# laclouis5/StructureDetector

Measured on AMD Instinct MI355X. Metric: images/sec (train fwd+bwd) and decode us/img at 512x512, higher is better.
Workload: dtype f32

## Files before the change

include/sdnet_hip.h:

```cpp
#ifndef SDNET_HIP_H
#define SDNET_HIP_H

#include <stddef.h>
#include <stdint.h>

#ifdef __cplusplus
extern "C" {
#endif

#define SD_ERR_INVALID   (-1)
#define SD_ERR_WORKSPACE (-2)
#define SD_ERR_ALIGN     (-3)

#define SD_MAX_TOPK 1024

typedef void* sd_stream_t;

int         sd_version(void);
const char* sd_last_error(void);
int         sd_build_flags(void);


int sd_clamped_sigmoid(const float* x, float* y, int64_t n, sd_stream_t stream);

// ... 198 lines not shown
int sd_loss_fwd_per_image(const sd_loss_desc* d, float* out, void* workspace, size_t workspace_bytes, sd_stream_t stream);

int sd_loss_bwd(const sd_loss_desc* d, const float* out8, const float* grad_out, float* dhead, sd_stream_t stream);



typedef struct sd_conv_desc {
    int B, Hi, Wi, Cin, Ho, Wo, Cout, R, S, stride, pad;
} sd_conv_desc;

size_t sd_conv2d_fwd_workspace_bytes(const sd_conv_desc* d);
int sd_conv2d_fwd(const float* x_nhwc, const float* w_krsc, float* y_nhwc, const sd_conv_desc* d,
                  const float* scale, const float* shift, const float* residual, int res_up2, int relu,
                  void* workspace, size_t workspace_bytes, sd_stream_t stream);
size_t sd_conv2d_stem_fwd_workspace_bytes(const sd_conv_desc* d);
int sd_conv2d_stem_fwd(const float* x_nchw, const float* w_krsc, void* y_nhwc, const sd_conv_desc* d,
                       const float* scale, const float* shift, int relu, int out_bf16, void* workspace,
                       size_t workspace_bytes, sd_stream_t stream);

int    sd_conv2d_fwd_sb_supported(const sd_conv_desc* d, int bf16);
size_t sd_conv2d_fwd_sb_workspace_bytes(const sd_conv_desc* d, int bf16);
size_t sd_conv2d_fwd_sb_state_bytes(const sd_conv_desc* d, int bf16);
int sd_conv2d_fwd_sb(const void* x_nhwc, const void* w_krsc, void* y_nhwc, const sd_conv_desc* d, const float* scale, const float* shift,
                     const void* residual, int res_up2, int relu, int bf16, void* workspace, size_t workspace_bytes, void* state,
                     size_t state_bytes, sd_stream_t stream);

size_t sd_conv2d_stem_fwd_bn_stats_workspace_bytes(const sd_conv_desc* d);
int sd_conv2d_stem_fwd_bn_stats(const float* x_nchw, const float* w, float* y, const sd_conv_desc* d, float eps, float momentum,
                                float* running_mean, float* running_var, float* mean, float* invstd, void* workspace,
                                size_t workspace_bytes, sd_stream_t stream);

size_t sd_conv2d_fwd_bn_stats_workspace_bytes(const sd_conv_desc* d);
int sd_conv2d_fwd_bn_stats(const float* x, const float* w, float* y, const sd_conv_desc* d, float eps, float momentum,
                           float* running_mean, float* running_var, float* mean, float* invstd, void* workspace,
                           size_t workspace_bytes, sd_stream_t stream);
int sd_bn_finalize_scratch_rows(int rows);
int sd_bn_finalize_stats(const float* partial, int rows, int64_t M, int C, float eps, float momentum, float* running_mean,
                         float* running_var, float* mean, float* invstd, float* scratch, sd_stream_t stream);

size_t sd_conv2d_dgrad_bn_reduce_workspace_bytes(const sd_conv_desc* d);
int sd_conv2d_dgrad_bn_reduce(const float* dy, const float* w_t, float* dx, const sd_conv_desc* d, const float* residual,
                              const float* bn_x, const float* bn_y, int relu, const float* mean, const float* invstd,
                              const float* gamma, const float* beta, float* dgamma, float* dbeta, int accumulate,
                              float* means_out, void* workspace, size_t workspace_bytes, sd_stream_t stream);
int sd_bn_bwd_finalize(const float* partial, int rows, int64_t M, int C, float* dgamma, float* dbeta, int accumulate,
                       float* means_out, float* scratch, sd_stream_t stream);
int sd_bn_bwd_apply(const float* dy, const float* x, const float* y, int relu, int64_t M, int C, const float* mean,
                    const float* invstd, const float* gamma, const float* beta, const float* means, float* dx, float* g_out,
                    sd_stream_t stream);

int sd_set_option(const char* name, int value);

const char* sd_conv2d_kernel_name(const sd_conv_desc* d, int pass);

int sd_cast_f32_to_bf16(const float* x, void* y_bf16, int64_t n, sd_stream_t stream);
size_t sd_conv2d_fwd_bf16_workspace_bytes(const sd_conv_desc* d);
int sd_conv2d_fwd_bf16(const void* x_nhwc_bf16, const void* w_krsc_bf16, void* y_nhwc_bf16, const sd_conv_desc* d,
                       const float* scale, const float* shift, const void* residual_bf16, int res_up2, int relu,
                       void* workspace, size_t workspace_bytes, sd_stream_t stream);
int sd_maxpool3x3s2_fwd_bf16(const void* x_bf16, void* y_bf16, int B, int Hi, int Wi, int C, sd_stream_t stream);
int sd_stem_bn_relu_maxpool_fwd_bf16(const float* x_nchw, const float* w, const float* scale, const float* shift, void* y_bf16,
                                     const sd_conv_desc* d, sd_stream_t stream);

int sd_cast_bf16_to_f32(const void* x_bf16, float* y, int64_t n, sd_stream_t stream);
size_t sd_conv2d_fwd_bf16_bn_stats_workspace_bytes(const sd_conv_desc* d);
int sd_conv2d_fwd_bf16_bn_stats(const void* x_nhwc_bf16, const void* w_krsc_bf16, void* y_nhwc_bf16, const sd_conv_desc* d, float eps,
                                float momentum, float* running_mean, float* running_var, float* mean, float* invstd,
                                void* workspace, size_t workspace_bytes, sd_stream_t stream);
int sd_conv2d_stem_fwd_bn_stats_bf16mm(const float* x_nchw, const float* w, float* y, const sd_conv_desc* d, float eps, float momentum,
                                       float* running_mean, float* running_var, float* mean, float* invstd,
                                       void* workspace, size_t workspace_bytes, sd_stream_t stream);
int sd_conv2d_stem_fwd_bn_stats_bf16(const float* x_nchw, const float* w, void* y_bf16, const sd_conv_desc* d, float eps, float momentum,
                                     float* running_mean, float* running_var, float* mean, float* invstd, void* workspace,
                                     size_t workspace_bytes, sd_stream_t stream);
int sd_bn_relu_maxpool_fwd_bf16(const void* x_bf16, int B, int Hi, int Wi, int C, const float* mean, const float* invstd, const float* gamma,
                                const float* beta, void* y_pool_bf16, uint8_t* idx, sd_stream_t stream);
int sd_maxpool_bn_relu_bwd_bf16(const void* dpool_bf16, const uint8_t* idx, const void* x_bf16, int B, int Hi, int Wi, int C, const float* mean,
                                const float* invstd, const float* gamma, const float* beta, float* dx, float* dgamma, float* dbeta, int accumulate,
                                void* workspace, size_t workspace_bytes, sd_stream_t stream);
int sd_maxpool_bn_relu_bwd_bf16_dx16(const void* dpool_bf16, const uint8_t* idx, const void* x_bf16, int B, int Hi, int Wi, int C, const float* mean,
                                     const float* invstd, const float* gamma, const float* beta, void* dx_bf16, float* dgamma, float* dbeta,
                                     int accumulate, void* workspace, size_t workspace_bytes, sd_stream_t stream);
int sd_conv2d_transpose_weights_bf16(const float* w, void* w_t_bf16, int Cout, int taps, int Cin, sd_stream_t stream);

int sd_conv2d_fwd_bf16_head_supported(const sd_conv_desc* d, int head_co);
size_t sd_head_split_bf16_bytes(void);
int sd_head_split_bf16(const float* head_w, const float* head_bias, int head_co, void* prepared, sd_stream_t stream);
int sd_conv2d_fwd_bf16_head(const void* x_bf16, const void* w_bf16, const sd_conv_desc* d, const float* scale, const float* shift, int relu,
                            const void* head_prepared, int head_co, float* head_y, sd_stream_t stream);
int sd_conv2d_dgrad_bf16(const void* dy_bf16, const void* w_t_bf16, void* dx_bf16, const sd_conv_desc* d, const void* residual_bf16,
                         int res_mode, sd_stream_t stream);
size_t sd_conv2d_wgrad_bf16_workspace_bytes(const sd_conv_desc* d);
int sd_conv2d_wgrad_bf16(const void* dy_bf16, const void* x_nhwc_bf16, float* dw_krsc, const sd_conv_desc* d, int accumulate,
                         void* workspace, size_t workspace_bytes, sd_stream_t stream);
int sd_bn_apply_bf16(const void* x, void* y, int64_t M, int C, const float* mean, const float* invstd, const float* gamma,
                     const float* beta, const void* residual, int relu, uint8_t* relu_mask_out, sd_stream_t stream);
int sd_bn_bwd_bf16(const void* dy, const void* x, const void* y, int relu, int64_t M, int C, const float* mean, const float* invstd,
                   const float* gamma, const float* beta, void* dx, void* g_out, float* dgamma, float* dbeta, int accumulate,
                   void* workspace, size_t workspace_bytes, sd_stream_t stream);
int sd_bn_train_stats_bf16(const void* x, int64_t M, int C, float eps, float momentum, float* running_mean, float* running_var,
                           float* mean, float* invstd, void* workspace, size_t workspace_bytes, sd_stream_t stream);
int sd_col_sum_bf16(const void* x, int64_t M, int C, float* out, int accumulate, void* workspace, size_t workspace_bytes, sd_stream_t stream);
int sd_upsample2x_bwd_bf16(const void* dy, const void* add, void* dx, int B, int H, int W, int C, sd_stream_t stream);
int sd_head_fwd_bf16(const void* x_nhwc_bf16, const float* w, const float* bias, float* y_nchw, int B, int HW, int C,
                     int Co, sd_stream_t stream);
int sd_conv2d_dgrad(const float* dy_nhwc, const float* w_t, float* dx_nhwc, const sd_conv_desc* d,
// ... 129 lines not shown
```

structuredetector_amd/_lib.py:

```python
from __future__ import annotations

import ctypes as C
import os
from pathlib import Path

import torch

_HERE = Path(__file__).resolve().parent
LIB_PATH = Path(os.environ.get("SDNET_HIP_LIB", _HERE / "csrc" / "libsdnet_hip.so"))

_lib = None

c_f32p = C.c_void_p
c_i64 = C.c_int64
c_int = C.c_int
c_float = C.c_float
c_size = C.c_size_t
c_vp = C.c_void_p


class SdError(RuntimeError):
    pass


# ... 104 lines not shown
    "sd_conv2d_fwd_sb": (c_int, [c_vp, c_vp, c_vp, C.POINTER(ConvDesc), c_vp, c_vp, c_vp, c_int, c_int, c_int, c_vp, c_size, c_vp, c_size, c_vp]),
    "sd_conv2d_stem_fwd_workspace_bytes": (c_size, [C.POINTER(ConvDesc)]),
    "sd_conv2d_stem_fwd": (c_int, [c_vp, c_vp, c_vp, C.POINTER(ConvDesc), c_vp, c_vp, c_int, c_int, c_vp, c_size, c_vp]),
    "sd_cast_f32_to_bf16": (c_int, [c_vp, c_vp, c_i64, c_vp]),
    "sd_conv2d_fwd_bf16_workspace_bytes": (c_size, [C.POINTER(ConvDesc)]),
    "sd_conv2d_fwd_bf16": (c_int, [c_vp, c_vp, c_vp, C.POINTER(ConvDesc), c_vp, c_vp, c_vp, c_int, c_int, c_vp, c_size, c_vp]),
    "sd_conv2d_fwd_bf16_head_supported": (c_int, [C.POINTER(ConvDesc), c_int]),
    "sd_head_split_bf16_bytes": (c_size, []),
    "sd_head_split_bf16": (c_int, [c_vp, c_vp, c_int, c_vp, c_vp]),
    "sd_conv2d_fwd_bf16_head": (c_int, [c_vp, c_vp, C.POINTER(ConvDesc), c_vp, c_vp, c_int, c_vp, c_int, c_vp, c_vp]),
    "sd_cast_bf16_to_f32": (c_int, [c_vp, c_vp, c_i64, c_vp]),
    "sd_conv2d_fwd_bf16_bn_stats_workspace_bytes": (c_size, [c_vp]),
    "sd_conv2d_fwd_bf16_bn_stats": (c_int, [c_vp, c_vp, c_vp, c_vp, c_float, c_float, c_vp, c_vp, c_vp, c_vp, c_vp, c_size, c_vp]),
    "sd_conv2d_wgrad_bf16_workspace_bytes": (c_size, [c_vp]),
    "sd_conv2d_wgrad_bf16": (c_int, [c_vp, c_vp, c_vp, c_vp, c_int, c_vp, c_size, c_vp]),
    "sd_conv2d_transpose_weights_bf16": (c_int, [c_vp, c_vp, c_int, c_int, c_int, c_vp]),
    "sd_conv2d_dgrad_bf16": (c_int, [c_vp, c_vp, c_vp, c_vp, c_vp, c_int, c_vp]),
    "sd_bn_apply_bf16": (c_int, [c_vp, c_vp, c_i64, c_int, c_vp, c_vp, c_vp, c_vp, c_vp, c_int, c_vp, c_vp]),
    "sd_bn_bwd_bf16": (c_int, [c_vp, c_vp, c_vp, c_int, c_i64, c_int, c_vp, c_vp, c_vp, c_vp, c_vp, c_vp, c_vp, c_vp, c_int, c_vp, c_size, c_vp]),
    "sd_bn_train_stats_bf16": (c_int, [c_vp, c_i64, c_int, c_float, c_float, c_vp, c_vp, c_vp, c_vp, c_vp, c_size, c_vp]),
    "sd_col_sum_bf16": (c_int, [c_vp, c_i64, c_int, c_vp, c_int, c_vp, c_size, c_vp]),
    "sd_upsample2x_bwd_bf16": (c_int, [c_vp, c_vp, c_vp, c_int, c_int, c_int, c_int, c_vp]),
    "sd_maxpool3x3s2_fwd_bf16": (c_int, [c_vp, c_vp, c_int, c_int, c_int, c_int, c_vp]),
    "sd_stem_bn_relu_maxpool_fwd_bf16": (c_int, [c_vp, c_vp, c_vp, c_vp, c_vp, c_vp, c_vp]),
    "sd_head_fwd_bf16": (c_int, [c_vp, c_vp, c_vp, c_vp, c_int, c_int, c_int, c_int, c_vp]),
    "sd_conv2d_dgrad": (c_int, [c_vp, c_vp, c_vp, C.POINTER(ConvDesc), c_vp, c_vp]),
    "sd_conv2d_transpose_weights": (c_int, [c_vp, c_vp, c_int, c_int, c_int, c_vp]),
    "sd_conv2d_transpose_weights_batched": (c_int, [c_vp, c_vp, c_vp, c_int, c_int, c_int, c_vp]),
    "sd_conv2d_wgrad_workspace_bytes": (c_size, [C.POINTER(ConvDesc)]),
    "sd_conv2d_wgrad": (c_int, [c_vp, c_vp, c_vp, C.POINTER(ConvDesc), c_int, c_vp, c_size, c_vp]),
    "sd_conv2d_stem_wgrad_workspace_bytes": (c_size, [C.POINTER(ConvDesc)]),
    "sd_conv2d_stem_wgrad": (c_int, [c_vp, c_vp, c_vp, C.POINTER(ConvDesc), c_int, c_vp, c_size, c_vp]),
    "sd_conv2d_stem_wgrad_bf16mm": (c_int, [c_vp, c_vp, c_vp, C.POINTER(ConvDesc), c_int, c_vp, c_size, c_vp]),
    "sd_conv2d_stem_wgrad_bf16": (c_int, [c_vp, c_vp, c_vp, C.POINTER(ConvDesc), c_int, c_vp, c_size, c_vp]),
    "sd_col_reduce_workspace_bytes": (c_size, [c_i64, c_int]),
    "sd_bn_train_stats": (c_int, [c_vp, c_i64, c_int, c_float, c_float, c_vp, c_vp, c_vp, c_vp, c_vp, c_size, c_vp]),
    "sd_bn_apply": (c_int, [c_vp, c_vp, c_i64, c_int, c_vp, c_vp, c_vp, c_vp, c_vp, c_int, c_vp, c_vp]),
    "sd_bn_fold": (c_int, [c_vp, c_vp, c_vp, c_vp, c_float, c_int, c_vp, c_vp, c_vp]),
    "sd_bn_bwd": (c_int, [c_vp, c_vp, c_vp, c_int, c_i64, c_int, c_vp, c_vp, c_vp, c_vp, c_vp, c_vp, c_vp, c_vp, c_int, c_vp, c_size, c_vp]),
    "sd_col_sum": (c_int, [c_vp, c_i64, c_int, c_vp, c_int, c_vp, c_size, c_vp]),
    "sd_maxpool3x3s2_fwd": (c_int, [c_vp, c_vp, c_vp, c_int, c_int, c_int, c_int, c_vp]),
    "sd_maxpool3x3s2_bwd": (c_int, [c_vp, c_vp, c_vp, c_int, c_int, c_int, c_int, c_vp]),
    "sd_upsample2x_bwd": (c_int, [c_vp, c_vp, c_vp, c_int, c_int, c_int, c_int, c_vp]),
    "sd_head_fwd": (c_int, [c_vp, c_vp, c_vp, c_vp, c_int, c_int, c_int, c_int, c_vp]),
    "sd_head_bwd_workspace_bytes": (c_size, [c_int] * 4),
    "sd_head_bwd": (c_int, [c_vp] * 6 + [c_int] * 5 + [c_vp, c_size, c_vp]),
    "sd_head_bwd_bf16": (c_int, [c_vp] * 6 + [c_int] * 5 + [c_vp, c_size, c_vp]),
    "sd_adam_step": (c_int, [c_vp, c_vp, c_vp, c_vp, c_i64, c_int, c_float, c_float, c_float, c_float, c_float, c_vp]),
    "sd_grad_sumsq_workspace_bytes": (c_size, [c_i64]),
    "sd_grad_sumsq": (c_int, [c_vp, c_i64, c_vp, c_size, c_vp]),
    "sd_optim_step": (c_int, [c_vp, c_vp, c_vp, c_vp, c_i64, c_int, c_float, c_float, c_float, c_float, c_float, c_float, c_vp, c_float, c_vp, c_int,
                              c_vp, c_float, c_vp, c_vp]),
    "sd_conv2d_kernel_name": (C.c_char_p, [c_vp, c_int]),
    "sd_set_option": (c_int, [C.c_char_p, c_int]),
    "sd_decode_set_option": (c_int, [C.c_char_p, c_int]),
    "sd_decode_kernel_names": (C.c_char_p, [c_int] * 9),
    "sd_conv2d_stem_fwd_bn_stats_workspace_bytes": (c_size, [c_vp]),
    "sd_conv2d_stem_fwd_bn_stats": (c_int, [c_vp, c_vp, c_vp, c_vp, c_float, c_float, c_vp, c_vp, c_vp, c_vp, c_vp, c_size, c_vp]),
    "sd_conv2d_stem_fwd_bn_stats_bf16mm": (c_int, [c_vp, c_vp, c_vp, c_vp, c_float, c_float, c_vp, c_vp, c_vp, c_vp, c_vp, c_size, c_vp]),
    "sd_conv2d_stem_fwd_bn_stats_bf16": (c_int, [c_vp, c_vp, c_vp, c_vp, c_float, c_float, c_vp, c_vp, c_vp, c_vp, c_vp, c_size, c_vp]),
    "sd_conv2d_dgrad_half_res": (c_int, [c_vp] * 6),
    "sd_bn_relu_maxpool_fwd": (c_int, [c_vp, c_int, c_int, c_int, c_int] + [c_vp] * 7),
    "sd_bn_relu_maxpool_fwd_bf16": (c_int, [c_vp, c_int, c_int, c_int, c_int] + [c_vp] * 7),
    "sd_maxpool_bn_relu_bwd": (c_int, [c_vp, c_vp, c_vp, c_int, c_int, c_int, c_int] + [c_vp] * 7 + [c_int, c_vp, c_size, c_vp]),
    "sd_maxpool_bn_relu_bwd_bf16": (c_int, [c_vp, c_vp, c_vp, c_int, c_int, c_int, c_int] + [c_vp] * 7 + [c_int, c_vp, c_size, c_vp]),
    "sd_maxpool_bn_relu_bwd_bf16_dx16": (c_int, [c_vp, c_vp, c_vp, c_int, c_int, c_int, c_int] + [c_vp] * 7 + [c_int, c_vp, c_size, c_vp]),
    "sd_conv2d_fwd_bn_stats_workspace_bytes": (c_size, [c_vp]),
    "sd_conv2d_fwd_bn_stats": (c_int, [c_vp, c_vp, c_vp, c_vp, c_float, c_float, c_vp, c_vp, c_vp, c_vp, c_vp, c_size, c_vp]),
    "sd_conv2d_dgrad_bn_reduce_workspace_bytes": (c_size, [c_vp]),
    "sd_conv2d_dgrad_bn_reduce": (c_int, [c_vp] * 5 + [c_vp, c_vp, c_int] + [c_vp] * 6 + [c_int, c_vp, c_vp, c_size, c_vp]),
    "sd_bn_bwd_finalize": (c_int, [c_vp, c_int, c_i64, c_int, c_vp, c_vp, c_int, c_vp, c_vp, c_vp]),
    "sd_bn_bwd_apply": (c_int, [c_vp, c_vp, c_vp, c_int, c_i64, c_int] + [c_vp] * 8),
    "sd_bn_finalize_scratch_rows": (c_int, [c_int]),
    "sd_bn_finalize_stats": (c_int, [c_vp, c_int, c_i64, c_int, c_float, c_float, c_vp, c_vp, c_vp, c_vp, c_vp, c_vp]),
    "sd_bn_stats_from_sums": (c_int, [c_vp, c_int, c_float, c_float, c_vp, c_vp, c_vp, c_vp, c_vp]),
    "sd_bn_bwd_means_from_sums": (c_int, [c_vp, c_int, c_vp, c_vp]),
    "sd_bn_stats_sums": (c_int, [c_vp, c_int, c_i64, c_int, c_vp, c_vp, c_vp]),
    "sd_bn_bwd_sums": (c_int, [c_vp, c_int, c_i64, c_int, c_vp, c_vp, c_int, c_vp, c_vp, c_vp]),
    "sd_bn_train_sums": (c_int, [c_vp, c_i64, c_int, c_vp, c_vp, c_size, c_vp]),
    "sd_bn_train_sums_bf16": (c_int, [c_vp, c_i64, c_int, c_vp, c_vp, c_size, c_vp]),
    "sd_conv2d_fwd_bn_stats_rows": (c_int, [c_vp, c_int]),
    "sd_conv2d_fwd_bn_sums": (c_int, [c_vp, c_vp, c_vp, c_vp, c_vp, c_vp, c_size, c_vp]),
    "sd_conv2d_fwd_bf16_bn_sums": (c_int, [c_vp, c_vp, c_vp, c_vp, c_vp, c_vp, c_size, c_vp]),
    "sd_conv2d_stem_fwd_bn_sums": (c_int, [c_vp, c_vp, c_vp, c_vp, c_vp, c_vp, c_size, c_vp]),
    "sd_conv2d_stem_fwd_bn_sums_bf16mm": (c_int, [c_vp, c_vp, c_vp, c_vp, c_vp, c_vp, c_size, c_vp]),
    "sd_conv2d_stem_fwd_bn_sums_bf16": (c_int, [c_vp, c_vp, c_vp, c_vp, c_vp, c_vp, c_size, c_vp]),
    "sd_conv2d_dgrad_bn_reduce_sums": (c_int, [c_vp, c_vp, c_vp, c_vp, c_vp, c_vp, c_vp, c_int] + [c_vp] * 6 + [c_int, c_vp, c_vp, c_size, c_vp]),
    "sd_bn_bwd_reduce": (c_int, [c_vp, c_vp, c_vp, c_int, c_i64, c_int] + [c_vp] * 6 + [c_int, c_vp, c_vp, c_size, c_vp]),
    "sd_bn_bwd_reduce_bf16": (c_int, [c_vp, c_vp, c_vp, c_int, c_i64, c_int] + [c_vp] * 6 + [c_int, c_vp, c_vp, c_size, c_vp]),
    "sd_bn_bwd_apply_bf16": (c_int, [c_vp, c_vp, c_vp, c_int, c_i64, c_int] + [c_vp] * 8),
    "sd_maxpool_bn_relu_bwd_reduce": (c_int, [c_vp, c_vp, c_vp, c_int, c_int, c_int, c_int] + [c_vp] * 6 + [c_int, c_vp, c_vp, c_size, c_vp]),
    "sd_maxpool_bn_relu_bwd_reduce_bf16": (c_int, [c_vp, c_vp, c_vp, c_int, c_int, c_int, c_int] + [c_vp] * 6 + [c_int, c_vp, c_vp, c_size, c_vp]),
    "sd_maxpool_bn_relu_bwd_apply": (c_int, [c_vp, c_vp, c_vp, c_int, c_int, c_int, c_int] + [c_vp] * 7),
    "sd_maxpool_bn_relu_bwd_apply_bf16": (c_int, [c_vp, c_vp, c_vp, c_int, c_int, c_int, c_int] + [c_vp] * 7),
    "sd_maxpool_bn_relu_bwd_apply_bf16_dx16": (c_int, [c_vp, c_vp, c_vp, c_int, c_int, c_int, c_int] + [c_vp] * 7),
    "sd_allreduce_unique_id": (c_int, [c_vp]),
    "sd_allreduce_init": (c_int, [c_vp, c_int, c_int, C.POINTER(c_vp)]),
    "sd_allreduce_run": (c_int, [c_vp, c_vp, c_i64, c_vp]),
    "sd_allreduce_destroy": (c_int, [c_vp]),
    "sd_mfma_bf16_stream_flops": (C.c_double, [c_int]),
    "sd_mfma_bf16_stream": (c_int, [c_vp, c_vp, c_int, c_vp]),
    "sd_comm_sim_copy": (c_int, [c_vp, c_vp, c_size, c_size, c_int, c_float, c_vp]),
    "sd_range_enabled": (c_int, []),
    "sd_range_library": (C.c_char_p, []),
    "sd_range_push": (c_int, [C.c_char_p]),
    "sd_range_pop": (c_int, []),
# ... 87 lines not shown
```

structuredetector_amd/csrc/sd_conv.hip:

```cpp
#include <string.h>
#include "sd_common.h"
#include "sd_mfma.h"
#include "sd_conv_rows.h"

#ifndef SD_S2_LPT
#define SD_S2_LPT 1
#endif
namespace sd {


#ifndef SD_IGEMM_DMA
#define SD_IGEMM_DMA 1
#endif
#ifndef SD_ABLATE_HOT
#define SD_ABLATE_HOT 0
#endif
#ifndef SD_ABLATE_STORE
#define SD_ABLATE_STORE 0
#endif
#ifndef SD_ABLATE_PATCH
#define SD_ABLATE_PATCH 0
#endif
#if SD_ABLATE_HOT || SD_ABLATE_STORE || SD_ABLATE_PATCH || defined(SD_PP_ABL) || defined(SD_RS_ABL)
#warning "timing-only ablation build: this libsdnet_hip.so computes WRONG RESULTS; the Python loader refuses it unless SDNET_ALLOW_ABLATION=1"
// ... 10 lines not shown
#if defined(SD_PP_ABL) || defined(SD_RS_ABL) || defined(SD_SB_ABL) || defined(SD_SHAPE_EXP) || defined(SD_W16_ABL) || defined(SD_SR_ABL) || defined(SD_SF_ABL)
#define SD_EXPERIMENT_FLAG 16
#else
#define SD_EXPERIMENT_FLAG 0
#endif
void sd_nn_set_pool_pair(int v);
extern "C" int sd_build_flags(void) { return (SD_ABLATE_HOT ? 1 : 0) | (SD_ABLATE_STORE ? 2 : 0) | (SD_ABLATE_PATCH ? 4 : 0) | SD_TRACE_FLAG | SD_EXPERIMENT_FLAG; }

#ifndef SD_SHAPE_EXP
#define SD_SHAPE_EXP 0
#else
#define SD_SHAPE_EXP_BUILD 1
#endif
__device__ __forceinline__ f32x16 mfma_shape_exp(bf16x8 a, bf16x8 b, f32x16 c) {
    f32x4 c0 = __builtin_shufflevector(c, c, 0, 1, 2, 3), c1 = __builtin_shufflevector(c, c, 4, 5, 6, 7);
    c0 = __builtin_amdgcn_mfma_f32_16x16x32_bf16(a, b, c0, 0, 0, 0);
    c1 = __builtin_amdgcn_mfma_f32_16x16x32_bf16(b, a, c1, 0, 0, 0);
    c[0] = c0[0]; c[1] = c0[1]; c[2] = c0[2]; c[3] = c0[3]; c[4] = c1[0]; c[5] = c1[1]; c[6] = c1[2]; c[7] = c1[3];
    return c;
}
#define SD_MFMA_BF16(BIT, a, b, c) (((SD_SHAPE_EXP) & (BIT)) ? mfma_shape_exp(a, b, c) : __builtin_amdgcn_mfma_f32_32x32x16_bf16(a, b, c, 0, 0, 0))

#ifndef SD_IGEMM_LATE_DMA
#define SD_IGEMM_LATE_DMA 0
#endif
constexpr int NBUF = 2;
constexpr int BM = 128, BK = 32, LDK = BK;

struct ConvArgs {
    const void* x;
    const void* w;
    void* y;
    const float* scale;
    const float* shift;
    const void* res;
    int B, Hi, Wi, Ck, Ho, Wo, Nn, R, S;
    int mul, div, off, rsign;
    int relu, res_up2;
    int M, nk, kchunks;
    int splits;
    float* part;
    const float* bn_x;
    const float* bn_y;
    const float *bn_mean, *bn_invstd, *bn_gamma, *bn_beta;
    int bn_relu;
    float* stat;
    int pt_tw_log2, pt_pw, pt_pieces, pt_rolling, pt_flip;
    int pt_strip_log2;
    int par;
    const uint16_t* head_w;
    const float* head_b;
    float* head_y;
    int head_co;
};

__device__ __attribute__((aligned(128))) float g_zero_line[64];


__device__ __forceinline__ void s2_tile(int bid, int nwg, int n_tiles, int off, int& cls, int& tq, int& n_idx, int& tile_m) {
    if (SD_S2_LPT && (nwg & 31) == 0) {
        const int xcd = bid & 7, pos = bid >> 3, per = nwg >> 5;
        const int k4 = pos / per, within = xcd * per + (pos - k4 * per);
        cls = (off & 1) ? (k4 == 0 ? 3 : k4 == 3 ? 0 : k4) : k4;
        tq = within / n_tiles; n_idx = within - tq * n_tiles;
    } else {
        const int tile = xcd_remap(bid, nwg), tm = tile / n_tiles;
        cls = tm & 3; tq = tm >> 2; n_idx = tile - tm * n_tiles;
    }
    tile_m = 4 * tq + cls;
}


__device__ __forceinline__ float f4c(const float4& v, int t) { return t == 0 ? v.x : (t == 1 ? v.y : (t == 2 ? v.z : v.w)); }

struct BnRed4 { float4 mu, is, ga, be, s, q; };
__device__ __forceinline__ void bnred4_init(BnRed4& b, const ConvArgs& p, int n) {
    b.mu = *reinterpret_cast<const float4*>(p.bn_mean + n); b.is = *reinterpret_cast<const float4*>(p.bn_invstd + n);
    b.ga = b.be = b.s = b.q = make_float4(0.f, 0.f, 0.f, 0.f);
    if (p.bn_relu == 2) { b.ga = *reinterpret_cast<const float4*>(p.bn_gamma + n); b.be = *reinterpret_cast<const float4*>(p.bn_beta + n); }
}
__device__ __forceinline__ void bnred4_add(BnRed4& b, const ConvArgs& p, float4 g, int64_t m, int n) {
    const int64_t i = m * p.Nn + n;
    const float4 xv = *reinterpret_cast<const float4*>(p.bn_x + i);
    const float4 xh = make_float4((xv.x - b.mu.x) * b.is.x, (xv.y - b.mu.y) * b.is.y, (xv.z - b.mu.z) * b.is.z, (xv.w - b.mu.w) * b.is.w);
    if (p.bn_relu == 1) {
        const float4 yy = *reinterpret_cast<const float4*>(p.bn_y + i);
        g.x = yy.x > 0.f ? g.x : 0.f; g.y = yy.y > 0.f ? g.y : 0.f; g.z = yy.z > 0.f ? g.z : 0.f; g.w = yy.w > 0.f ? g.w : 0.f;
    } else if (p.bn_relu == 3) {
        const uint8_t mb = reinterpret_cast<const uint8_t*>(p.bn_y)[i >> 2];
        g.x = (mb & 1) ? g.x : 0.f; g.y = (mb & 2) ? g.y : 0.f; g.z = (mb & 4) ? g.z : 0.f; g.w = (mb & 8) ? g.w : 0.f;
    } else if (p.bn_relu == 2) {
        g.x = (xh.x * b.ga.x + b.be.x) > 0.f ? g.x : 0.f; g.y = (xh.y * b.ga.y + b.be.y) > 0.f ? g.y : 0.f;
        g.z = (xh.z * b.ga.z + b.be.z) > 0.f ? g.z : 0.f; g.w = (xh.w * b.ga.w + b.be.w) > 0.f ? g.w : 0.f;
    }
    b.s.x += g.x; b.s.y += g.y; b.s.z += g.z; b.s.w += g.w;
    b.q.x += g.x * xh.x; b.q.y += g.y * xh.y; b.q.z += g.z * xh.z; b.q.w += g.w * xh.w;
}
template <int LPR>
__device__ __forceinline__ void bnred4_wave_sum(BnRed4& b) {
#pragma unroll
    for (int o = LPR; o < 64; o <<= 1) {
        b.s.x += __shfl_xor(b.s.x, o); b.s.y += __shfl_xor(b.s.y, o); b.s.z += __shfl_xor(b.s.z, o); b.s.w += __shfl_xor(b.s.w, o);
        b.q.x += __shfl_xor(b.q.x, o); b.q.y += __shfl_xor(b.q.y, o); b.q.z += __shfl_xor(b.q.z, o); b.q.w += __shfl_xor(b.q.w, o);
    }
}

#define SD_BNRED_TERM(v, m, n, S, Q)                                                               \
    {                                                                                              \
        const float xv_ = p.bn_x[(int64_t)(m) * p.Nn + (n)];                                       \
        const float xh_ = (xv_ - bmu) * bis;                                                       \
        float g_ = (v);                                                                            \
        if (p.bn_relu == 1) g_ = p.bn_y[(int64_t)(m) * p.Nn + (n)] > 0.f ? g_ : 0.f;               \
        else if (p.bn_relu == 3) g_ = ((reinterpret_cast<const uint8_t*>(p.bn_y)[((int64_t)(m) * p.Nn + (n)) >> 2] >> ((n) & 3)) & 1) ? g_ : 0.f; \
        else if (p.bn_relu == 2) g_ = (xh_ * bga + bbe) > 0.f ? g_ : 0.f;                          \
        S += g_; Q += g_ * xh_;                                                                    \
    }

template <int BN, int MODE, bool BF16 = false>
__global__ __launch_bounds__(256, 2) void k_conv_igemm(ConvArgs p) {
    constexpr bool STEM = (MODE == 1);
    using T = typename std::conditional<BF16, uint16_t, float>::type;
    constexpr int KE = BF16 ? 64 : 32;
    constexpr int VE = BF16 ? 8 : 4;
    const T* const px_ = reinterpret_cast<const T*>(p.x);
    const T* const pw_ = reinterpret_cast<const T*>(p.w);
    const T* const zero_ = reinterpret_cast<const T*>(g_zero_line);
    constexpr int NT = BN / 64;
    __shared__ __attribute__((aligned(16))) float As0[BM * LDK];
    __shared__ __attribute__((aligned(16))) float As1[BM * LDK];
    __shared__ __attribute__((aligned(16))) float Bs0[BN * LDK];
    __shared__ __attribute__((aligned(16))) float Bs1[BN * LDK];
    __shared__ int orow[BM];
    __shared__ int rrow[BM];

    const int tid = threadIdx.x, lane = tid & 63, wave = tid >> 6;
    const int n_tiles = p.Nn / BN;
    const int tile = xcd_remap(blockIdx.x, gridDim.x);
    int tile_m = tile / n_tiles;
    int n0 = (tile % n_tiles) * BN;
    int m0 = tile_m * BM;

    int r0 = 0, s0 = 0, tstep = 1, nk = p.nk;
    int cls_base = 0, py = 0, px = 0;
    if (MODE == 2) {
        int cls, tq, n_idx;
        s2_tile(blockIdx.x, gridDim.x, n_tiles, p.off, cls, tq, n_idx, tile_m);
        n0 = n_idx * BN;
        const int Mq = p.M >> 2;
        cls_base = cls * Mq; m0 = cls_base + tq * BM;
        py = cls >> 1; px = cls & 1;
        r0 = (py + p.off) & 1; s0 = (px + p.off) & 1; tstep = 2;
        nk = ((p.R - r0 + 1) >> 1) * ((p.S - s0 + 1) >> 1) * p.kchunks;
    }

    const int srow = tid >> 3, sk = (tid & 7) * 4;
    const int ske = (tid & 7) * VE;
    const int img_stride = p.Hi * p.Wi * (STEM ? 3 : p.Ck);
#define SD_ROW_SETUP(i)                                                                           \
    int aty##i = 0, atx##i = 0;                                                                   \
    const T* aptr##i = px_;                                                                       \
    bool aok##i;                                                                                  \
    {                                                                                             \
        const int m = m0 + srow + 32 * i;                                                         \
        int pix = -1;                                                                             \
        aok##i = m < p.M;                                                                         \
        if (aok##i) {                                                                             \
            int ox, oy, b;                                                                        \
            if (MODE == 2) {                                                                      \
                const int ml = m - cls_base, hw = p.Wo >> 1, hh = p.Ho >> 1;                      \
                const int qx = ml % hw, t = ml / hw, qy = t % hh;                                 \
                b = t / hh; oy = 2 * qy + py; ox = 2 * qx + px;                                   \
            } else {                                                                              \
                ox = m % p.Wo; const int t = m / p.Wo; oy = t % p.Ho; b = t / p.Ho;               \
            }                                                                                     \
            aty##i = oy * p.mul + p.off;                                                          \
            atx##i = ox * p.mul + p.off;                                                          \
            aptr##i = px_ + (int64_t)b * img_stride;                                              \
            pix = (b * p.Ho + oy) * p.Wo + ox;                                                    \
            if ((tid & 7) == 0)       \
                rrow[srow + 32 * i] = (p.res_up2 == 2 && ((ox | oy) & 1)) ? -1 : (b * (p.Ho >> 1) + (oy >> 1)) * (p.Wo >> 1) + (ox >> 1); \
        }                                                                                         \
        if ((tid & 7) == 0) orow[srow + 32 * i] = pix;                                            \
    }
    SD_ROW_SETUP(0) SD_ROW_SETUP(1) SD_ROW_SETUP(2) SD_ROW_SETUP(3)
#undef SD_ROW_SETUP
    const int wk = p.R * p.S * (STEM ? 3 : p.Ck);
// ... 4285 lines not shown
    r.x = (const uint16_t*)a.x; r.w = (const uint16_t*)a.w; r.y = (uint16_t*)a.y; r.scale = a.scale; r.shift = a.shift;
    r.res = (const uint16_t*)a.res; r.stat = a.stat; r.relu = a.relu; r.flip = a.rsign < 0;
    return true;
}

static thread_local int g_rows16 = 1;
static bool conv_rows16_args(const RowsArgs& r) { return g_rows16 && !r.stat; }

static thread_local int g_rowsf32_min_units = 192;
static thread_local int g_stem_fwd_blocks = 512;
static bool conv_rowsf32_geometry(const ConvArgs& a, int mode, RowsArgsF& r) {
    if (mode != 0 || a.Ck != 64 || a.Nn != 64 || a.R != 3 || a.S != 3 || a.mul != 1 || a.div != 1 || a.splits > 1) return false;
    if (!((a.rsign == 1 && a.off == -1) || (a.rsign == -1 && a.off == 1))) return false;
    if (a.Ho != a.Hi || a.Wo != a.Wi || a.Wo % 64 || a.res_up2 || a.bn_x) return false;
    r = RowsArgsF{};
    r.B = a.B; r.H = a.Ho; r.W = a.Wo; r.segs = a.Wo / 64;
    const int cols = r.B * r.segs;
    r.rows = std::min(r.H, std::max(8, cdiv(r.H * cols, 256)));
    r.units_per_col = cdiv(r.H, r.rows);
    r.nunits = cols * r.units_per_col;
    if (r.nunits < g_rowsf32_min_units || (g_rowsf32_min_units > 1 && r.rows < 16)) return false;
    r.x = (const float*)a.x; r.w = (const float*)a.w; r.y = (float*)a.y; r.scale = a.scale; r.shift = a.shift;
    r.res = (const float*)a.res; r.stat = a.stat; r.relu = a.relu; r.flip = a.rsign < 0;
    return true;
}

static thread_local int g_pp_min_tiles = 200;
static thread_local int g_pp_strips = 1;
static bool conv_pp_geometry(ConvArgs& a, int mode, int min_tiles) {
    if (a.Nn % 128 || a.M % PP_BM || (a.M / PP_BM) * (a.Nn / 128) < min_tiles || a.res_up2) return false;
    a.pt_strip_log2 = 0;
    int l2 = 0;
    while ((1 << l2) < a.Wo) ++l2;
    if (g_pp_strips && (1 << l2) == a.Wo && a.Wo >= 128 && a.Wo <= 4096 && a.Ho % 4 == 0) {
        if (!SD_CONV_PATCH || mode != 0 || a.R != 3 || a.S != 3 || a.mul != 1 || a.div != 1 || a.splits > 1) return false;
        if (!((a.rsign == 1 && a.off == -1) || (a.rsign == -1 && a.off == 1))) return false;
        if (a.Ho != a.Hi || a.Wo != a.Wi || a.Ck % 32) return false;
        a.pt_tw_log2 = 6; a.pt_strip_log2 = l2 - 6; a.pt_rolling = 0; a.pt_pw = 66; a.pt_pieces = cdiv(6 * 66, 16); a.pt_flip = a.rsign < 0;
        return true;
    }
    return conv_patch_geometry(a, 128, mode, true, false, 1) && !a.pt_rolling;
}

static thread_local int g_stem_fwd_ring = 1;
static thread_local int g_igemm_big_bf16 = 0;
static int igemm_big_tiles(const ConvArgs& a, int BN, int mode) {
    if (!SD_IGEMM_BIG || (BN != 128 && !SD_IGEMM_BIG64 && !(SD_IGEMM_BIG64_S2 && mode == 2)) || (mode != 0 && mode != 2) || a.splits > 1) return 0;
    if (a.R * a.S * a.Ck < 512) return 0;
    const int m_per = mode == 2 ? a.M / 4 : a.M;
    const int big_tiles = (mode == 2 ? 4 : 1) * cdiv(m_per, BMB) * (a.Nn / BN);
    return (big_tiles >= 512 && (mode != 2 || m_per % BMB == 0)) ? big_tiles : 0;
}

enum ConvFamily {
    CONV_STREAM1X1,
    CONV_ROWS16,
    CONV_ROWS_BF16,
    CONV_ROWS_F32,
    CONV_PP,
    CONV_PP_HEAD,
    CONV_PATCH,
    CONV_PATCH_ROLL,
    CONV_IGEMM_BIG,
    CONV_IGEMM,
};

struct ConvPlan {
    ConvFamily family;
    bool bf16;
    int BN, mode;
    int grid_x, grid_y, block;
    size_t lds;
    int stat_rows;
    ConvArgs a;
    RowsArgs ra;
    RowsArgsF rf;
};

static ConvPlan plan_conv(const ConvArgs& a, bool bf16, bool stem = false) {
    ConvPlan p{};
    p.bf16 = bf16;
    p.a = a;
    p.BN = (a.Nn % 128 == 0) ? 128 : 64;
    p.mode = stem ? 1 : (a.par ? 2 : (a.div > 1 ? 3 : 0));
    p.grid_y = 1; p.block = 256;
    if (!stem && bf16) {
        if (conv1x1_stream_geometry(a, p.mode) && conv1x1_stream_args(a)) {
            p.family = CONV_STREAM1X1;
            p.grid_x = std::min(512, cdiv(a.M / (a.Ck == 64 ? 32 : 16), 4));
            return p;
        }
        if (conv_rows64_geometry(a, p.mode, p.ra)) {
            p.family = conv_rows16_args(p.ra) ? CONV_ROWS16 : CONV_ROWS_BF16;
            p.grid_x = std::min(p.ra.nunits, 256); p.lds = RS_LDS_BYTES; p.stat_rows = p.ra.nunits;
            return p;
        }
        ConvArgs t = a;
        if (conv_pp_geometry(t, p.mode, g_pp_min_tiles)) {
            p.a = t;
            p.family = a.head_y ? CONV_PP_HEAD : CONV_PP;
            p.BN = 128; p.grid_x = (a.M / PP_BM) * (a.Nn / 128); p.block = 512; p.lds = PP_LDS_FLOATS * sizeof(float); p.stat_rows = a.M / PP_BM;
            return p;
        }
    }
    if (!stem && !bf16 && conv_rowsf32_geometry(a, p.mode, p.rf)) {
        p.family = CONV_ROWS_F32;
        p.grid_x = std::min(p.rf.nunits, 256); p.lds = RF_LDS_BYTES; p.stat_rows = p.rf.nunits;
        return p;
    }
    if (!stem) {
        if (const int PBN = patch_tile_bn(p.a, p.BN, p.mode, bf16)) {
            p.family = p.a.pt_rolling ? CONV_PATCH_ROLL : CONV_PATCH;
            p.BN = PBN; p.grid_x = (a.M / BMB) * (a.Nn / PBN); p.stat_rows = cdiv(a.M, BMB);
            return p;
        }
    }
    if (const int big_tiles = (!bf16 || (g_igemm_big_bf16 && p.BN == 128)) ? igemm_big_tiles(a, p.BN, p.mode) : 0) {
        p.family = CONV_IGEMM_BIG;
        p.grid_x = big_tiles; p.stat_rows = cdiv(a.M, BMB);
        return p;
    }
    p.family = CONV_IGEMM;
    p.grid_x = cdiv(a.M, BM) * (a.Nn / p.BN); p.grid_y = a.splits > 1 ? a.splits : 1; p.stat_rows = a.splits > 1 ? 0 : cdiv(a.M, BM);
    return p;
}

static const char* conv_plan_name(const ConvPlan& p, char* buf, size_t n) {
    const char* tf = p.bf16 ? "true" : "false";
    switch (p.family) {
    case CONV_STREAM1X1: return p.a.Ck == 64 ? "k_conv1x1_stream_bf16<64, 2>" : "k_conv1x1_stream_bf16<128, 1>";
    case CONV_ROWS16: return "k_conv3x3_c64_rows16_bf16";
    case CONV_ROWS_BF16: return "k_conv3x3_c64_rows_bf16";
    case CONV_ROWS_F32: return "k_conv3x3_c64_rows_f32";
    case CONV_PP: return "k_conv3x3_bf16_pp";
    case CONV_PP_HEAD: return "k_conv3x3_bf16_pp_head";
    case CONV_PATCH: snprintf(buf, n, "k_conv3x3_patch<%d, %s>", p.BN, tf); return buf;
    case CONV_PATCH_ROLL: snprintf(buf, n, "k_conv3x3_patch_roll<%d, %s>", p.BN, tf); return buf;
    case CONV_IGEMM_BIG: snprintf(buf, n, "k_conv_igemm_big<%d, %d, %s>", p.BN, p.mode, tf); return buf;
    case CONV_IGEMM: snprintf(buf, n, "k_conv_igemm<%d, %d, %s>", p.BN, p.mode, tf); return buf;
    }
    return "";
}

template <auto KERNEL>
static int raise_dynamic_lds(size_t bytes) {
    static thread_local bool raised = false;
    if (!raised) {
        SD_HIP(hipFuncSetAttribute(reinterpret_cast<const void*>(KERNEL), hipFuncAttributeMaxDynamicSharedMemorySize, (int)bytes));
        raised = true;
    }
    return 0;
}

template <int BN, int MODE, bool BF16 = false>
static void launch_tiles(const ConvPlan& p, hipStream_t st) {
    if constexpr ((BN == 128 || (!BF16 && (SD_IGEMM_BIG64 || (SD_IGEMM_BIG64_S2 && MODE == 2)))) && (MODE == 0 || MODE == 2)) {
        if (p.family == CONV_IGEMM_BIG) {
            hipLaunchKernelGGL((k_conv_igemm_big<BN, MODE, BF16>), dim3(p.grid_x), dim3(256), 0, st, p.a);
            return;
        }
    }
    hipLaunchKernelGGL((k_conv_igemm<BN, MODE, BF16>), dim3(p.grid_x, p.grid_y), dim3(256), 0, st, p.a);
}
template <int BN, bool BF16>
static void launch_tiles_mode(const ConvPlan& p, hipStream_t st) {
    if (p.mode == 0) launch_tiles<BN, 0, BF16>(p, st);
    else if (p.mode == 2) launch_tiles<BN, 2, BF16>(p, st);
    else launch_tiles<BN, 3, BF16>(p, st);
}
template <bool BF16>
static void launch_patch(const ConvPlan& p, hipStream_t st) {
    if (p.family == CONV_PATCH_ROLL) {
        if (p.BN == 128) hipLaunchKernelGGL((k_conv3x3_patch_roll<128, BF16>), dim3(p.grid_x), dim3(256), 0, st, p.a);
        else hipLaunchKernelGGL((k_conv3x3_patch_roll<64, BF16>), dim3(p.grid_x), dim3(256), 0, st, p.a);
    } else if (p.BN == 128) hipLaunchKernelGGL((k_conv3x3_patch<128, BF16>), dim3(p.grid_x), dim3(256), 0, st, p.a);
    else hipLaunchKernelGGL((k_conv3x3_patch<64, BF16>), dim3(p.grid_x), dim3(256), 0, st, p.a);
// ... 856 lines not shown
    a.x = dy; a.w = w_t; a.y = dx; a.res = residual;
    a.bn_x = bn_x; a.bn_y = bn_y; a.bn_relu = relu; a.bn_mean = mean; a.bn_invstd = invstd; a.bn_gamma = gamma; a.bn_beta = beta;
    a.stat = (float*)workspace;
    const ConvPlan p = plan_conv(a, false);
    if (int e = launch_plan(p, (hipStream_t)stream)) return e;
    const int rows = p.stat_rows;
    if (sums) return sd_bn_bwd_sums((const float*)workspace, rows, (int64_t)a.M, d->Cin, dgamma, dbeta, accumulate, sums,
                                    (float*)workspace + (size_t)rows * 2 * d->Cin, stream);
    return sd_bn_bwd_finalize((const float*)workspace, rows, (int64_t)a.M, d->Cin, dgamma, dbeta, accumulate, means_out,
                              (float*)workspace + (size_t)rows * 2 * d->Cin, stream);
}

int sd_conv2d_dgrad_bn_reduce(const float* dy, const float* w_t, float* dx, const sd_conv_desc* d, const float* residual, const float* bn_x,
                              const float* bn_y, int relu, const float* mean, const float* invstd, const float* gamma, const float* beta,
                              float* dgamma, float* dbeta, int accumulate, float* means_out, void* workspace, size_t workspace_bytes,
                              sd_stream_t stream) {
    SD_REQUIRE(means_out, SD_ERR_INVALID, "sd_conv2d_dgrad_bn_reduce: null pointer");
    return conv_dgrad_bn_reduce_any("sd_conv2d_dgrad_bn_reduce", dy, w_t, dx, d, residual, bn_x, bn_y, relu, mean, invstd, gamma, beta, dgamma, dbeta,
                                    accumulate, means_out, nullptr, workspace, workspace_bytes, stream);
}

int sd_conv2d_dgrad_bn_reduce_sums(const float* dy, const float* w_t, float* dx, const sd_conv_desc* d, const float* residual, const float* bn_x,
                                   const float* bn_y, int relu, const float* mean, const float* invstd, const float* gamma, const float* beta,
                                   float* dgamma, float* dbeta, int accumulate, double* sums, void* workspace, size_t workspace_bytes,
                                   sd_stream_t stream) {
    SD_REQUIRE(sums, SD_ERR_INVALID, "sd_conv2d_dgrad_bn_reduce_sums: null pointer");
    return conv_dgrad_bn_reduce_any("sd_conv2d_dgrad_bn_reduce_sums", dy, w_t, dx, d, residual, bn_x, bn_y, relu, mean, invstd, gamma, beta, dgamma,
                                    dbeta, accumulate, nullptr, sums, workspace, workspace_bytes, stream);
}

#ifdef SD_PP_TRACE
int sd_debug_pp_trace(unsigned long long* out32) { return (int)hipMemcpyFromSymbol(out32, HIP_SYMBOL(sd::g_pp_trace), sizeof(unsigned long long) * 64); }
int sd_debug_stem_trace(unsigned long long* out64) { return (int)hipMemcpyFromSymbol(out64, HIP_SYMBOL(sd::g_stem_trace), sizeof(unsigned long long) * 64); }
int sd_debug_pp_timeline(unsigned long long* out, int blocks) { return (int)hipMemcpyFromSymbol(out, HIP_SYMBOL(sd::g_pp_tl), sizeof(unsigned long long) * 4 * (blocks < 4096 ? blocks : 4096)); }
#endif

int sd_set_option(const char* name, int value) {
    if (name && !strcmp(name, "conv_patch_min_tiles")) { g_patch_min_tiles = value; return 0; }
    if (name && !strcmp(name, "conv_patch_bn64")) { g_patch_bn64 = value; return 0; }
    if (name && !strcmp(name, "conv_pp_min_tiles")) { g_pp_min_tiles = value; return 0; }
    if (name && !strcmp(name, "conv1x1_stream_min_pixels")) { g_conv1x1_stream_min_px = value; return 0; }
    if (name && !strcmp(name, "igemm_big_bf16")) { g_igemm_big_bf16 = value; return 0; }
    if (name && !strcmp(name, "stem_fwd_ring")) { g_stem_fwd_ring = value; return 0; }
    if (name && !strcmp(name, "pool_fwd_pair")) { sd_nn_set_pool_pair(value); return 0; }
    if (name && !strcmp(name, "wgrad_bf16_ring")) { g_wgrad_bf16_ring = value; return 0; }
    if (name && !strcmp(name, "wgrad_f32_ring")) { g_wgrad_f32_ring = value; return 0; }
    if (name && !strcmp(name, "conv_pp_strips")) { g_pp_strips = value; return 0; }
    if (name && !strcmp(name, "conv_patch_narrow")) { g_patch_narrow = value; return 0; }
    if (name && !strcmp(name, "conv_fwd_split_k")) { g_fwd_split_k = value; return 0; }
    if (name && !strcmp(name, "conv_rows64_min_units")) { g_rows64_min_units = value; return 0; }
    if (name && !strcmp(name, "conv_rows16")) { g_rows16 = value; return 0; }
    if (name && !strcmp(name, "conv_rows_f32_min_units")) { g_rowsf32_min_units = value; return 0; }
    if (name && !strcmp(name, "stem_fwd_blocks")) { g_stem_fwd_blocks = value; return 0; }
    sd::set_error("sd_set_option: unknown option '%s'", name ? name : "(null)");
    return SD_ERR_INVALID;
}

const char* sd_conv2d_kernel_name(const sd_conv_desc* d, int pass) {
    static thread_local char name[64];
    if (!d || d->Cin <= 0 || d->Cout <= 0) return "";
    if (pass == 2) {
        const WgradPlan p = plan_wgrad(d, false);
        switch (p.family) {
        case WGRAD_TAPS_RING2: return "k_wgrad3x3_ring2";
        case WGRAD_TAPS_RING: return "k_wgrad3x3_ring";
        case WGRAD_TAPS: return p.roww == 32 ? "k_wgrad3x3<32>" : "k_wgrad3x3<16>";
        default: snprintf(name, sizeof(name), "k_conv_wgrad<%d, %d>", p.TN, p.TC); return name;
        }
    }
    return conv_plan_name(plan_query(d, pass & 15, (pass & 16) != 0, false), name, sizeof(name));
}

}
```

Measured before the change: 875.0.

## Add persistent weight-resident streaming path for f32 1x1 conv igemm

```diff
diff --git a/include/sdnet_hip.h b/include/sdnet_hip.h
--- a/include/sdnet_hip.h
+++ b/include/sdnet_hip.h
@@ -274,6 +274,8 @@
 int sd_set_option(const char* name, int value);
 
 const char* sd_conv2d_kernel_name(const sd_conv_desc* d, int pass);
+
+int sd_conv2d_fwd_streams_1x1(const sd_conv_desc* d, int pass);
 
 int sd_cast_f32_to_bf16(const float* x, void* y_bf16, int64_t n, sd_stream_t stream);
 size_t sd_conv2d_fwd_bf16_workspace_bytes(const sd_conv_desc* d);
diff --git a/structuredetector_amd/_lib.py b/structuredetector_amd/_lib.py
--- a/structuredetector_amd/_lib.py
+++ b/structuredetector_amd/_lib.py
@@ -180,6 +180,7 @@
     "sd_optim_step": (c_int, [c_vp, c_vp, c_vp, c_vp, c_i64, c_int, c_float, c_float, c_float, c_float, c_float, c_float, c_vp, c_float, c_vp, c_int,
                               c_vp, c_float, c_vp, c_vp]),
     "sd_conv2d_kernel_name": (C.c_char_p, [c_vp, c_int]),
+    "sd_conv2d_fwd_streams_1x1": (c_int, [c_vp, c_int]),
     "sd_set_option": (c_int, [C.c_char_p, c_int]),
     "sd_decode_set_option": (c_int, [C.c_char_p, c_int]),
     "sd_decode_kernel_names": (C.c_char_p, [c_int] * 9),
diff --git a/structuredetector_amd/csrc/sd_conv.hip b/structuredetector_amd/csrc/sd_conv.hip
--- a/structuredetector_amd/csrc/sd_conv.hip
+++ b/structuredetector_amd/csrc/sd_conv.hip
@@ -86,6 +86,7 @@
     const float* head_b;
     float* head_y;
     int head_co;
+    int stream_run;
 };
 
 __device__ __attribute__((aligned(128))) float g_zero_line[64];
@@ -149,6 +150,169 @@
         else if (p.bn_relu == 2) g_ = (xh_ * bga + bbe) > 0.f ? g_ : 0.f;                          \
         S += g_; Q += g_ * xh_;                                                                    \
     }
+
+template <int MI>
+__device__ __forceinline__ void stream_res_request(const ConvArgs& p, int m_base, int col, int (&rm)[MI], float4 (&rv)[MI][MI][4]) {
+    const float* const res = reinterpret_cast<const float*>(p.res);
+#pragma unroll
+    for (int mi = 0; mi < MI; ++mi) {
+        const int m = m_base + mi * 32;
+        rm[mi] = m;
+        if (p.res_up2) {
+            const int ox = m % p.Wo, tt = m / p.Wo, oy = tt % p.Ho, b = tt / p.Ho;
+            rm[mi] = (p.res_up2 == 2 && ((ox | oy) & 1)) ? -1 : (b * (p.Ho >> 1) + (oy >> 1)) * (p.Wo >> 1) + (ox >> 1);
+        }
+        const float* rp = res ? res + (rm[mi] >= 0 ? (int64_t)rm[mi] * p.Nn : 0) + col : g_zero_line + (col & 4);
+#pragma unroll
+        for (int ni = 0; ni < MI; ++ni)
+#pragma unroll
+            for (int g = 0; g < 4; ++g) rv[mi][ni][g] = *reinterpret_cast<const float4*>(rp + ni * 32 + 8 * g);
+    }
+}
+template <int MI>
+__device__ __forceinline__ void stream_tile_store(const ConvArgs& p, f32x16 (&acc)[MI][MI], int m_base, int col, int lcol, const int (&rm)[MI],
+                                                  const float4 (&rv)[MI][MI][4], uint32_t sc_a, uint32_t sh_a) {
+    float* const y = reinterpret_cast<float*>(p.y);
+#pragma unroll
+    for (int mi = 0; mi < MI; ++mi) {
+        const int m = m_base + mi * 32;
+#pragma unroll
+        for (int ni = 0; ni < MI; ++ni) {
+#pragma unroll
+            for (int gp = 0; gp < 2; ++gp) {
+                const uint32_t nl0 = (lcol + ni * 32 + 16 * gp) * 4;
+                f32x4 sc0 = lds_read128_async<0>(sc_a + nl0), sc1 = lds_read128_async<32>(sc_a + nl0);
+                f32x4 sh0 = lds_read128_async<0>(sh_a + nl0), sh1 = lds_read128_async<32>(sh_a + nl0);
+                SD_LDS_WAIT4(0, sc0, sc1, sh0, sh1);
+#pragma unroll
+                for (int gq = 0; gq < 2; ++gq) {
+                    const int g = 2 * gp + gq;
+                    const f32x4 sc4 = gq ? sc1 : sc0, sh4 = gq ? sh1 : sh0;
+                    float4 v = make_float4(acc[mi][ni][4 * g], acc[mi][ni][4 * g + 1], acc[mi][ni][4 * g + 2], acc[mi][ni][4 * g + 3]);
+                    v.x = v.x * sc4[0] + sh4[0]; v.y = v.y * sc4[1] + sh4[1]; v.z = v.z * sc4[2] + sh4[2]; v.w = v.w * sc4[3] + sh4[3];
+                    if (p.res && rm[mi] >= 0) { const float4 r = rv[mi][ni][g]; v.x += r.x; v.y += r.y; v.z += r.z; v.w += r.w; }
+                    if (p.relu) { v.x = fmaxf(v.x, 0.f); v.y = fmaxf(v.y, 0.f); v.z = fmaxf(v.z, 0.f); v.w = fmaxf(v.w, 0.f); }
+                    *reinterpret_cast<float4*>(y + (int64_t)m * p.Nn + col + ni * 32 + 8 * g) = v;
+                }
+            }
+        }
+    }
+#pragma unroll
+    for (int mi = 0; mi < MI; ++mi)
+#pragma unroll
+        for (int ni = 0; ni < MI; ++ni)
+#pragma unroll
+            for (int e = 0; e < 16; ++e) acc[mi][ni][e] = 0.f;
+}
+
+template <int BN>
+__device__ __forceinline__ void conv1x1_stream_f32(const ConvArgs& p, float* S0, float* S1, float* W0, float* W1, float* sc_lds, float* sh_lds) {
+    constexpr int TM = BN;
+    constexpr int NST = (BN / 64) * (BN / 64) * 4;
+    constexpr int MI = BN / 64;
+    constexpr int RI = TM / 32;
+    constexpr int WCH = BN * LDK;
+    const float* const x = reinterpret_cast<const float*>(p.x);
+    const float* const w = reinterpret_cast<const float*>(p.w);
+    const int tid = threadIdx.x, lane = tid & 63, wave = __builtin_amdgcn_readfirstlane(tid >> 6);
+    const int n_tiles = p.Nn / BN;
+    const int run_idx = blockIdx.x / n_tiles, n0 = (blockIdx.x - run_idx * n_tiles) * BN;
+    const int t0 = run_idx * p.stream_run, t1 = min(t0 + p.stream_run, p.M / TM);
+    const int nk = p.nk;
+    const int srow = tid >> 3;
+    const int qe = ((tid & 7) ^ ((srow >> 1) & 7)) * 4;
+
+    for (int c = 0; c < nk; ++c) {
+        float* wd = ((c & 1) ? W1 : W0) + (c >> 1) * WCH;
+#pragma unroll
+        for (int i = 0; i < RI; ++i) lds_dma16(w + (int64_t)(n0 + srow + 32 * i) * p.Ck + c * BK + qe, wd + (32 * i + 8 * wave) * LDK);
+    }
+#define SD_ST_ISSUE(ST, T, C)                                                                     \
+    _Pragma("unroll") for (int i = 0; i < RI; ++i)                                                \
+        lds_dma16(x + (int64_t)((T) * TM + srow + 32 * i) * p.Ck + (C) * BK + qe, (ST) + (32 * i + 8 * wave) * LDK);
+
+    const int wm0 = (wave >> 1) * (32 * MI), wn0 = (wave & 1) * (32 * MI);
+    const int fr = lane & 31, fh = lane >> 5;
+    const int rd_swz = (fr >> 1) & 7;
+    f32x16 acc[MI][MI];
+#pragma unroll
+    for (int mi = 0; mi < MI; ++mi)
+#pragma unroll
+        for (int ni = 0; ni < MI; ++ni)
+#pragma unroll
+            for (int e = 0; e < 16; ++e) acc[mi][ni][e] = 0.f;
+
+    if (tid < BN) {
+        sc_lds[tid] = p.scale ? p.scale[n0 + tid] : 1.f;
+        sh_lds[tid] = p.shift ? p.shift[n0 + tid] : 0.f;
+    }
+    const uint32_t sc_a = lds_addr(sc_lds), sh_a = lds_addr(sh_lds);
+    if (t0 < t1) { SD_ST_ISSUE(S0, t0, 0) }
+    __syncthreads();
+
+#define SD_ST_SLOT(ks) ((((ks) * 2 + fh) ^ rd_swz) << 2)
+#define SD_ST_COMPUTE(XB, WB)                                                                                     \
+    {                                                                                                             \
+        const float* Xb = (XB) + (wm0 + fr) * LDK;                                                                \
+        const float* Wb = (WB) + (wn0 + fr) * LDK;                                                                \
+        float4 nx0 = *reinterpret_cast<const float4*>(Xb + SD_ST_SLOT(0)), nx1 = nx0;                             \
+        float4 nw0 = *reinterpret_cast<const float4*>(Wb + SD_ST_SLOT(0)), nw1 = nw0;                             \
+        if (MI == 2) {                                                                                            \
+            nx1 = *reinterpret_cast<const float4*>(Xb + 32 * LDK + SD_ST_SLOT(0));                                \
+            nw1 = *reinterpret_cast<const float4*>(Wb + 32 * LDK + SD_ST_SLOT(0));                                \
+        }                                                                                                         \
+        _Pragma("unroll") for (int ks = 0; ks < BK / 8; ++ks) {                                                   \
+            const float4 x0 = nx0, x1 = nx1, w0 = nw0, w1 = nw1;                                                  \
+            if (ks + 1 < BK / 8) {                                                                                \
+                nx0 = *reinterpret_cast<const float4*>(Xb + SD_ST_SLOT(ks + 1));                                  \
+                nw0 = *reinterpret_cast<const float4*>(Wb + SD_ST_SLOT(ks + 1));                                  \
+                if (MI == 2) {                                                                                    \
+                    nx1 = *reinterpret_cast<const float4*>(Xb + 32 * LDK + SD_ST_SLOT(ks + 1));                   \
+                    nw1 = *reinterpret_cast<const float4*>(Wb + 32 * LDK + SD_ST_SLOT(ks + 1));                   \
+                }                                                                                                 \
+            }                                                                                                     \
+            __builtin_amdgcn_sched_barrier(0);            \
+            _Pragma("unroll") for (int t = 0; t < 4; ++t) {                                                       \
+                acc[0][0] = __builtin_amdgcn_mfma_f32_32x32x2f32(f4c(w0, t), f4c(x0, t), acc[0][0], 0, 0, 0);     \
+                if (MI == 2) {                                                                                    \
+                    acc[MI - 1][0] = __builtin_amdgcn_mfma_f32_32x32x2f32(f4c(w0, t), f4c(x1, t), acc[MI - 1][0], 0, 0, 0);           \
+                    acc[0][MI - 1] = __builtin_amdgcn_mfma_f32_32x32x2f32(f4c(w1, t), f4c(x0, t), acc[0][MI - 1], 0, 0, 0);           \
+                    acc[MI - 1][MI - 1] = __builtin_amdgcn_mfma_f32_32x32x2f32(f4c(w1, t), f4c(x1, t), acc[MI - 1][MI - 1], 0, 0, 0); \
+                }                                                                                                 \
+            }                                                                                                     \
+            __builtin_amdgcn_sched_barrier(0);                                                                    \
+        }                                                                                                         \
+    }
+
+    for (int t = t0; t < t1; ++t) {
+        int c = 0;
+        for (; c + 2 < nk; c += 2) {
+            SD_ST_ISSUE(S1, t, c + 1)
+            SD_ST_COMPUTE(S0, W0 + (c >> 1) * WCH)
+            __syncthreads();
+            SD_ST_ISSUE(S0, t, c + 2)
+            SD_ST_COMPUTE(S1, W1 + (c >> 1) * WCH)
+            __syncthreads();
+        }
+        SD_ST_ISSUE(S1, t, c + 1)
+        SD_ST_COMPUTE(S0, W0 + (c >> 1) * WCH)
+        __syncthreads();
+        int rm[MI];
+        float4 rv[MI][MI][4];
+        const int m_base = t * TM + wm0 + fr, lcol = wn0 + 4 * fh;
+        stream_res_request<MI>(p, m_base, n0 + lcol, rm, rv);
+        if (t + 1 < t1) { SD_ST_ISSUE(S0, t + 1, 0) }
+        SD_ST_COMPUTE(S1, W1 + (c >> 1) * WCH)
+        stream_tile_store<MI>(p, acc, m_base, n0 + lcol, lcol, rm, rv, sc_a, sh_a);
+        __builtin_amdgcn_sched_barrier(0);
+        wait_vmcnt_and_lds<NST>();
+        __builtin_amdgcn_s_barrier();
+        __builtin_amdgcn_sched_barrier(0);
+    }
+#undef SD_ST_COMPUTE
+#undef SD_ST_SLOT
+#undef SD_ST_ISSUE
+}
 
 template <int BN, int MODE, bool BF16 = false>
 __global__ __launch_bounds__(256, 2) void k_conv_igemm(ConvArgs p) {
@@ -164,8 +328,17 @@
     __shared__ __attribute__((aligned(16))) float As1[BM * LDK];
     __shared__ __attribute__((aligned(16))) float Bs0[BN * LDK];
     __shared__ __attribute__((aligned(16))) float Bs1[BN * LDK];
-    __shared__ int orow[BM];
-    __shared__ int rrow[BM];
+    __shared__ __attribute__((aligned(16))) int orow[BM];
+    __shared__ __attribute__((aligned(16))) int rrow[BM];
+
+    if constexpr (MODE == 0 && !BF16) {
+        if (p.stream_run > 0) {
+            float* const sc_lds = reinterpret_cast<float*>(orow), * const sh_lds = reinterpret_cast<float*>(rrow);
+            if constexpr (BN == 128) conv1x1_stream_f32<BN>(p, As0, As1, Bs0, Bs1, sc_lds, sh_lds);
+            else conv1x1_stream_f32<BN>(p, Bs0, Bs1, As0, As1, sc_lds, sh_lds);
+            return;
+        }
+    }
 
     const int tid = threadIdx.x, lane = tid & 63, wave = tid >> 6;
     const int n_tiles = p.Nn / BN;
@@ -4557,6 +4730,15 @@
     return (big_tiles >= 512 && (mode != 2 || m_per % BMB == 0)) ? big_tiles : 0;
 }
 
+static thread_local int g_conv1x1_stream_f32 = 1;
+static int conv1x1_stream_f32_run(const ConvArgs& a, int BN, int mode) {
+    if (!g_conv1x1_stream_f32 || mode != 0 || a.R != 1 || a.S != 1 || a.mul != 1 || a.div != 1 || a.off != 0) return 0;
+    if (a.Ho != a.Hi || a.Wo != a.Wi || a.splits > 1 || a.stat || a.bn_x || a.M % 128) return 0;
+    if (a.Ck % (2 * BK) || (size_t)a.Ck * BN > (size_t)2 * BM * LDK) return 0;
+    const int mt = a.M / BN, slots = std::max(1, (BN == 128 ? 512 : 768) / (a.Nn / BN));
+    return std::max(cdiv(mt, slots), std::min(4, mt));
+}
+
 enum ConvFamily {
     CONV_STREAM1X1,
     CONV_ROWS16,
@@ -4627,6 +4809,10 @@
     }
     p.family = CONV_IGEMM;
     p.grid_x = cdiv(a.M, BM) * (a.Nn / p.BN); p.grid_y = a.splits > 1 ? a.splits : 1; p.stat_rows = a.splits > 1 ? 0 : cdiv(a.M, BM);
+    if (const int run = (!bf16 && !stem) ? conv1x1_stream_f32_run(a, p.BN, p.mode) : 0) {
+        p.a.stream_run = run;
+        p.grid_x = cdiv(a.M / p.BN, run) * (a.Nn / p.BN);
+    }
     return p;
 }
 
@@ -5589,6 +5775,7 @@
     if (name && !strcmp(name, "conv_rows16")) { g_rows16 = value; return 0; }
     if (name && !strcmp(name, "conv_rows_f32_min_units")) { g_rowsf32_min_units = value; return 0; }
     if (name && !strcmp(name, "stem_fwd_blocks")) { g_stem_fwd_blocks = value; return 0; }
+    if (name && !strcmp(name, "conv1x1_stream_f32")) { g_conv1x1_stream_f32 = value; return 0; }
     sd::set_error("sd_set_option: unknown option '%s'", name ? name : "(null)");
     return SD_ERR_INVALID;
 }
@@ -5608,4 +5795,11 @@
     return conv_plan_name(plan_query(d, pass & 15, (pass & 16) != 0, false), name, sizeof(name));
 }
 
-}
+int sd_conv2d_fwd_streams_1x1(const sd_conv_desc* d, int pass) {
+    if (!d || d->B <= 0 || d->Cin <= 0 || d->Cout <= 0 || (pass != 0 && pass != 1)) return 0;
+    if ((pass == 0 ? d->Cin % 32 || d->Cout % 64 : d->Cout % 32 || d->Cin % 64)) return 0;
+    const ConvPlan p = plan_query(d, pass, false, false);
+    return p.family == CONV_IGEMM ? p.a.stream_run : 0;
+}
+
+}
```

Result: no change. 877.3 (median of 6 runs) (+0.3%).
